# mkshing/e4t-diffusion

Hardware: AMD Instinct MI355X
Metric: E4T pretrain images/sec @512px bf16 (higher is better)
Workload: dtype bf16; 1 GPU; SD-1.4 UNet + ViT-H-14 E4T encoder pretrain step, 512px; per_gpu_batch=16, global_batch=16, parallelism=dp1, trainable=weight offsets + E4T head (ViT frozen), next_batch_prefetch=vit+vae

## Files before the change

e4t-diffusion_amd/csrc/common.h:

```cpp
#pragma once
#include <hip/hip_runtime.h>
#include <stdint.h>
#include <stdio.h>
#include <string.h>

typedef uint16_t bf16_t;

typedef __attribute__((ext_vector_type(8))) __bf16 bf16x8;
typedef __attribute__((ext_vector_type(4))) __bf16 bf16x4;
typedef __attribute__((ext_vector_type(16))) float f32x16;
typedef __attribute__((ext_vector_type(4))) float f32x4;

#define E4T_WAVE 64

typedef __attribute__((ext_vector_type(4))) short s16x4;
__device__ __forceinline__ bf16x8 tr_frag(const uint16_t* lds_lo, const uint16_t* lds_hi) {
  union { s16x4 h[2]; bf16x8 v; } u;
  u.h[0] = __builtin_amdgcn_ds_read_tr16_b64_v4i16((__attribute__((address_space(3))) s16x4*)lds_lo);
  u.h[1] = __builtin_amdgcn_ds_read_tr16_b64_v4i16((__attribute__((address_space(3))) s16x4*)lds_hi);
  return u.v;
}

extern "C" __attribute__((visibility("hidden"))) void e4t_set_error(const char* msg);
#define E4T_FAIL(code, ...)                                  \
  do {                                                       \
    char _b[512];                                            \
    snprintf(_b, sizeof(_b), __VA_ARGS__);                   \
    e4t_set_error(_b);                                       \
    return (code);                                           \
  } while (0)
#define E4T_REQUIRE(cond, ...) \
  do {                         \
    if (!(cond)) E4T_FAIL(-22, __VA_ARGS__); \
  } while (0)
#define E4T_CHECK_LAUNCH(name)                                                    \
  do {                                                                            \
    hipError_t _e = hipGetLastError();                                            \
    if (_e != hipSuccess) E4T_FAIL(-5, "%s: %s", name, hipGetErrorString(_e));    \
  } while (0)

extern "C" __attribute__((visibility("hidden"))) int e4t_launch_log_enabled(void);
extern "C" __attribute__((visibility("hidden"))) void e4t_launch_logf(const char* fmt, ...);
#define E4T_LOG_LAUNCH(...)                                          \
  do {                                                               \
    if (e4t_launch_log_enabled()) e4t_launch_logf(__VA_ARGS__);      \
  } while (0)

__device__ __forceinline__ float bf2f(bf16_t v) { return __uint_as_float(((uint32_t)v) << 16); }
typedef __attribute__((ext_vector_type(2))) __bf16 bf16x2_native;
typedef __attribute__((ext_vector_type(2))) float f32x2_native;
__device__ __forceinline__ bf16_t f2bf(float f) {
  const __bf16 b = (__bf16)f;
  bf16_t u;
  __builtin_memcpy(&u, &b, 2);
  return u;
}
__device__ __forceinline__ uint32_t pack2bf(float lo, float hi) {
  const f32x2_native f = {lo, hi};
  const bf16x2_native v = __builtin_convertvector(f, bf16x2_native);
  uint32_t u;
  __builtin_memcpy(&u, &v, 4);
  return u;
}
__device__ __forceinline__ float bflo(uint32_t w) { return __uint_as_float(w << 16); }
__device__ __forceinline__ float bfhi(uint32_t w) { return __uint_as_float(w & 0xffff0000u); }

__device__ __forceinline__ void unpack8(const uint4& v, float* f) {
  f[0] = bflo(v.x); f[1] = bfhi(v.x); f[2] = bflo(v.y); f[3] = bfhi(v.y);
  f[4] = bflo(v.z); f[5] = bfhi(v.z); f[6] = bflo(v.w); f[7] = bfhi(v.w);
}
__device__ __forceinline__ uint4 pack8(const float* f) {
  uint4 v;
  v.x = pack2bf(f[0], f[1]); v.y = pack2bf(f[2], f[3]); v.z = pack2bf(f[4], f[5]); v.w = pack2bf(f[6], f[7]);
  return v;
}
__device__ __forceinline__ void unpack4(const uint2& v, float* f) {
  f[0] = bflo(v.x); f[1] = bfhi(v.x); f[2] = bflo(v.y); f[3] = bfhi(v.y);
}
__device__ __forceinline__ uint2 pack4(const float* f) {
  uint2 v;
  v.x = pack2bf(f[0], f[1]); v.y = pack2bf(f[2], f[3]);
  return v;
}

__device__ __forceinline__ float wave_sum(float v) {
#pragma unroll
  for (int o = 32; o > 0; o >>= 1) v += __shfl_xor(v, o, 64);
  return v;
}
__device__ __forceinline__ float wave_max(float v) {
#pragma unroll
  for (int o = 32; o > 0; o >>= 1) v = fmaxf(v, __shfl_xor(v, o, 64));
  return v;
}
__device__ __forceinline__ float block_sum(float v, float* red) {
  v = wave_sum(v);
  const int w = threadIdx.x >> 6, nw = (blockDim.x + 63) >> 6;
  __syncthreads();
  if ((threadIdx.x & 63) == 0) red[w] = v;
  __syncthreads();
  float t = 0.f;
  for (int i = 0; i < nw; ++i) t += red[i];
  return t;
}

typedef __attribute__((ext_vector_type(4))) unsigned u32x4_native;
__device__ __forceinline__ uint4 buf_load16(__amdgpu_buffer_rsrc_t rs, unsigned voff, int soff) {
  const u32x4_native v = __builtin_amdgcn_raw_buffer_load_b128(rs, voff, soff, 0);
  return make_uint4(v.x, v.y, v.z, v.w);
}
__device__ __forceinline__ __amdgpu_buffer_rsrc_t make_rsrc(const void* base, unsigned bytes) {
  return __builtin_amdgcn_make_buffer_rsrc((void*)base, 0, (int)bytes, 0x00020000);
}

__device__ __forceinline__ float silu_f(float x) { return x / (1.f + __expf(-x)); }
__device__ __forceinline__ float dsilu_f(float x) {
  const float s = 1.f / (1.f + __expf(-x));
  return s * (1.f + x * (1.f - s));
}
__device__ __forceinline__ float erf_pos(float z, float e) {
  const float t = __builtin_amdgcn_rcpf(fmaf(0.3275911f, z, 1.f));
  float q = 1.061405429f;
  q = fmaf(q, t, -1.453152027f);
  q = fmaf(q, t, 1.421413741f);
  q = fmaf(q, t, -0.284496736f);
  q = fmaf(q, t, 0.254829592f);
  return fmaf(-q * t, e, 1.f);
}
__device__ __forceinline__ float gelu_f(float x) {
  const float e = __expf(-0.5f * x * x);
  const float er = erf_pos(fabsf(x) * 0.70710678118654752f, e);
  return 0.5f * x * (1.f + copysignf(er, x));
}
__device__ __forceinline__ float dgelu_f(float x) {
  const float e = __expf(-0.5f * x * x);
  const float er = erf_pos(fabsf(x) * 0.70710678118654752f, e);
  const float cdf = 0.5f * (1.f + copysignf(er, x));
  return fmaf(x * 0.39894228040143268f, e, cdf);
}

__device__ __forceinline__ float geglu_f(float a, float g) { return a * gelu_f(g); }
__device__ __forceinline__ float geglu_da_f(float d, float g) { return d * gelu_f(g); }
__device__ __forceinline__ float geglu_dg_f(float d, float a, float g) { return d * a * dgelu_f(g); }

static inline int cdiv(int a, int b) { return (a + b - 1) / b; }
static inline long long cdivl(long long a, long long b) { return (a + b - 1) / b; }
```

e4t-diffusion_amd/csrc/gemm.hip:

```cpp
#include "gemm_common.h"

namespace {


template <int BM, int BN, int WGM, int WGN, int MODE>
__global__ __launch_bounds__(256) void gemm_kernel(GemmArgs p) {
  constexpr int WM = BM / WGM, WN = BN / WGN;
  constexpr int FM = WM / 32, FN = WN / 32;
  constexpr int NA = BM * (BK / 8) / 256;
  constexpr int NB = BN * (BK / 8) / 256;
  static_assert(WGM * WGN == 4, "4 waves per workgroup");
  static_assert(NA >= 1 && NB >= 1, "tile too small");

  __shared__ __attribute__((aligned(16))) bf16_t smem[(BM + BN) * LDS_LD];
  bf16_t* const As = smem;
  bf16_t* const Bs = smem + BM * LDS_LD;

  const int tid = threadIdx.x;
  const int lane = tid & 63, wave = tid >> 6;
  const int wm = wave / WGN, wn = wave % WGN;
  const int m0 = blockIdx.y * BM, n0 = blockIdx.x * BN;

  const KRange kr = batch_entry<BK>(p, (p.K + BK - 1) / BK);
  const int kt_begin = kr.begin, kt_end = kr.end;
// ... 608 lines not shown
  wb.init(kt_begin, BK);
  int b_so = 0;
  int a_ky = (kt_begin % 9) / 3, a_chb = (kt_begin / 9) * BK * 2;
  auto issue_b = [&](bool hi, bf16_t* dst) __attribute__((always_inline)) {
    if (!hi) b_so = cm_b_so(p, wb);
    else b_so = __builtin_amdgcn_readfirstlane(b_so + HK * 2);
#pragma unroll
    for (int j = 0; j < 2; ++j) buf_dma16(rs_b, b_vo[j], b_so, dst + (wave * 32 + j * 16) * HK);
    if (hi) wb.next(BK);
  };
  auto issue_strip = [&](bool hi, bf16_t* dst) __attribute__((always_inline)) {
    const int iy = y + a_ky - 1;
    const int so = __builtin_amdgcn_readfirstlane((int)((((long long)ib * p.Hin + iy + 1) * p.Win + x0) * p.Cin * 2) + a_chb + (hi ? HK * 2 : 0));
#pragma unroll
    for (int i = 0; i < 3; ++i)
      buf_dma16(rs_a, a_vo[i] | (unsigned)__builtin_amdgcn_sbfe(a_inv[i], (unsigned)a_ky, 1u), so, dst + (wave + 8 * i) * 512);
    if (hi && ++a_ky == 3) { a_ky = 0; a_chb += BK * 2; }
  };
  auto issue_strip_piece = [&](auto Ic, bool last, bf16_t* dst_lo) __attribute__((always_inline)) {
    constexpr int i = decltype(Ic)::value;
    const int iy = y + a_ky - 1;
    const int so = __builtin_amdgcn_readfirstlane((int)((((long long)ib * p.Hin + iy + 1) * p.Win + x0) * p.Cin * 2) + a_chb);
    const unsigned vo = a_vo[i] | (unsigned)__builtin_amdgcn_sbfe(a_inv[i], (unsigned)a_ky, 1u);
    buf_dma16(rs_a, vo, so, dst_lo + (wave + 8 * i) * 512);
    buf_dma16(rs_a, vo, so + HK * 2, dst_lo + HSTRIP + (wave + 8 * i) * 512);
    if (last && ++a_ky == 3) { a_ky = 0; a_chb += BK * 2; }
  };

  f32x16 acc[4][2];
#pragma unroll
  for (int i = 0; i < 4; ++i)
#pragma unroll
    for (int j = 0; j < 2; ++j)
#pragma unroll
      for (int r = 0; r < 16; ++r) acc[i][j][r] = 0.f;

  const int frow = lane & 31, fhi = lane >> 5;
  int a_off[3][4][2], b_off[2][2];
#pragma unroll
  for (int ks = 0; ks < 2; ++ks) {
#pragma unroll
    for (int kx = 0; kx < 3; ++kx)
#pragma unroll
      for (int i = 0; i < 4; ++i) {
        const int o = wr * 128 + i * 32 + frow;
        const int r = sg.frag_row(o, kx);
        a_off[kx][i][ks] = frag_off<HK>(r, ks, fhi);
      }
#pragma unroll
    for (int j = 0; j < 2; ++j) {
      const int r = wc * 64 + j * 32 + frow;
      b_off[j][ks] = frag_off<HK>(r, ks, fhi);
    }
  }
  bf16_t* const Bq = smem + A_EL;
  issue_strip(false, smem);
  issue_strip(true, smem + HSTRIP);
  issue_b(false, Bq);
  issue_b(true, Bq + QUART);
  if (kt_begin + 1 < kt_end) issue_b(false, Bq + 2 * QUART);
  wait_vmcnt<0>();
  __builtin_amdgcn_s_barrier();

  bf16x8 af[2][2], bfr[2][2];
  using I0 = std::integral_constant<int, 0>; using I1 = std::integral_constant<int, 1>;
  using I2 = std::integral_constant<int, 2>; using I3 = std::integral_constant<int, 3>;
  auto phase = [&](auto Bc, auto Pc, auto ALLc, auto KXc, auto SPc, int kt) {
    constexpr int bb = decltype(Bc)::value, ph = decltype(Pc)::value, KX = decltype(KXc)::value, SP = decltype(SPc)::value;
    constexpr bool ALL = decltype(ALLc)::value;
    constexpr int kh = ph >> 1, mh = ph & 1;
    const bf16_t* const qa = smem + (2 * SP + kh) * HSTRIP;
    const bf16_t* const qb = Bq + (2 * bb + kh) * QUART;
#pragma unroll
    for (int i = 0; i < 2; ++i)
#pragma unroll
      for (int ks = 0; ks < 2; ++ks) af[i][ks] = *(const bf16x8*)(qa + a_off[KX][mh * 2 + i][ks]);
    if (mh == 0) {
#pragma unroll
      for (int j = 0; j < 2; ++j)
#pragma unroll
        for (int ks = 0; ks < 2; ++ks) bfr[j][ks] = *(const bf16x8*)(qb + b_off[j][ks]);
    }
    bool staged = true;
    if (ph == 0)      { staged = ALL || kt + 1 < kt_end; if (staged) issue_b(true, Bq + (2 * (bb ^ 1) + 1) * QUART); }
    else if (ph == 2) { staged = ALL || kt + 2 < kt_end; if (staged) issue_b(false, Bq + (2 * bb + 0) * QUART); }
    else if (4 * KX + ph == 1) { staged = ALL || kt + 3 < kt_end; if (staged) issue_strip_piece(I0{}, false, smem + 2 * (SP ^ 1) * HSTRIP); }
    else if (4 * KX + ph == 3) { staged = ALL || kt + 3 < kt_end; if (staged) issue_strip_piece(I1{}, false, smem + 2 * (SP ^ 1) * HSTRIP); }
    else if (4 * KX + ph == 5) { staged = ALL || kt + 2 < kt_end; if (staged) issue_strip_piece(I2{}, true, smem + 2 * (SP ^ 1) * HSTRIP); }
    constexpr int G_ = 4 * KX + ph;
    constexpr int NW_ = G_ == 0 ? 4 : G_ <= 2 ? 6 : G_ <= 6 ? 8 : G_ <= 8 ? 6 : 4;
    if (ALL || staged) wait_vmcnt<NW_>(); else wait_vmcnt<0>();
    __builtin_amdgcn_sched_barrier(0);
    __builtin_amdgcn_s_barrier();
    __builtin_amdgcn_sched_barrier(0);
    __builtin_amdgcn_s_setprio(1);
#pragma unroll
    for (int ks = 0; ks < 2; ++ks)
#pragma unroll
      for (int i = 0; i < 2; ++i)
#pragma unroll
        for (int j = 0; j < 2; ++j)
          acc[mh * 2 + i][j] = __builtin_amdgcn_mfma_f32_32x32x16_bf16(af[i][ks], bfr[j][ks], acc[mh * 2 + i][j], 0, 0, 0);
    __builtin_amdgcn_s_setprio(0);
    __builtin_amdgcn_sched_barrier(0);
    __builtin_amdgcn_s_barrier();
    __builtin_amdgcn_sched_barrier(0);
  };
  auto ktile = [&](auto Bc, auto KXc, auto SPc, auto ALLc, int kt) __attribute__((always_inline)) {
    phase(Bc, I0{}, ALLc, KXc, SPc, kt); phase(Bc, I1{}, ALLc, KXc, SPc, kt); phase(Bc, I2{}, ALLc, KXc, SPc, kt); phase(Bc, I3{}, ALLc, KXc, SPc, kt);
  };

  if (wr == 1) __builtin_amdgcn_s_barrier();
  {
    using YES = std::true_type; using NO = std::false_type;
    int kt = kt_begin;
    for (; kt + 8 <= kt_end; kt += 6) {
      ktile(I0{}, I0{}, I0{}, YES{}, kt);     ktile(I1{}, I1{}, I0{}, YES{}, kt + 1); ktile(I0{}, I2{}, I0{}, YES{}, kt + 2);
      ktile(I1{}, I0{}, I1{}, YES{}, kt + 3); ktile(I0{}, I1{}, I1{}, YES{}, kt + 4); ktile(I1{}, I2{}, I1{}, YES{}, kt + 5);
    }
    if (kt < kt_end) { ktile(I0{}, I0{}, I0{}, NO{}, kt); ktile(I1{}, I1{}, I0{}, NO{}, kt + 1); ktile(I0{}, I2{}, I0{}, NO{}, kt + 2); kt += 3; }
    if (kt < kt_end) { ktile(I1{}, I0{}, I1{}, NO{}, kt); ktile(I0{}, I1{}, I1{}, NO{}, kt + 1); ktile(I1{}, I2{}, I1{}, NO{}, kt + 2); kt += 3; }
  }
  if (wr == 0) __builtin_amdgcn_s_barrier();
  __syncthreads();
  write_tile<64, 64, 2, 2, GENERAL>(p, *(f32x16(*)[2][2])(acc + 0), wave_stage<64, 64>(smem, wave), lane, m0 + wr * 128, n0 + wc * 64);
  __syncthreads();
  write_tile<64, 64, 2, 2, GENERAL>(p, *(f32x16(*)[2][2])(acc + 2), wave_stage<64, 64>(smem, wave), lane, m0 + wr * 128 + 64, n0 + wc * 64);
}
static bool conv_pps_ok(const GemmArgs& p, int , int batch) {
  return strips_enabled() && p.mode == E4T_CONV_S1 && p.chan_major && batch == 1 && strip_rows_ok(p) && p.Wout == p.Win && p.Hout == p.Hin && p.Cin % 64 == 0 &&
         p.K == 9 * p.Cin && p.ktiles_per_split % 3 == 0 && p.M % 256 == 0;
}

template <int MODE, int BN, bool GENERAL>
__global__ __launch_bounds__(512) void gemm_pq_kernel(GemmArgs p) {
  constexpr int EPI = EPI_PLAIN;
#include "gemm_pq_kernel.inc"
}
template <int BN, int EPI>
__global__ __launch_bounds__(512) void gemm_pq_geglu_kernel(GemmArgs p) {
  constexpr int MODE = 0;
  constexpr bool GENERAL = false;
#include "gemm_pq_kernel.inc"
}

#ifdef PP_TRACE
}
extern "C" int e4t_debug_pp_trace(unsigned long long* out) {
  return (int)hipMemcpyFromSymbol(out, HIP_SYMBOL(g_pp_trace), sizeof(g_pp_trace));
}
namespace {
#endif

__global__ __launch_bounds__(512) void gemm_tn_kernel(GemmArgs p) {
  constexpr int BM = 128, BN = 128, WGN = 2, WM = 32, WN = 64, FN = 2;
  constexpr int OPER = BK * 128;
  constexpr int TILE = 2 * OPER;
  __shared__ __attribute__((aligned(16))) bf16_t smem[2 * TILE];

  const int tid = threadIdx.x;
  const int lane = tid & 63, wave = __builtin_amdgcn_readfirstlane(tid >> 6);
  const int wm = wave / WGN, wn = wave % WGN;
  int tile_x, tile_y, sz = blockIdx.z;
  if (p.xcd3) { xcd_tile3(tile_x, tile_y, sz); p.zslab = sz; }
  else xcd_tile(tile_x, tile_y, p.group_m);
  const int m0 = tile_y * BM, n0 = tile_x * BN;

  const int nkt = (p.K + BK - 1) / BK;
  const int kt_begin = sz * p.ktiles_per_split;
  int kt_end = kt_begin + p.ktiles_per_split;
  if (kt_end > nkt) kt_end = nkt;

  const __amdgpu_buffer_rsrc_t rs_a = __builtin_amdgcn_make_buffer_rsrc((void*)p.A, 0, (int)p.a_bytes, 0x00020000);
  const __amdgpu_buffer_rsrc_t rs_b = __builtin_amdgcn_make_buffer_rsrc((void*)p.B, 0, (int)p.b_bytes, 0x00020000);
  const int prow = lane >> 4, pchunk = lane & 15;
  const int lchunk = (((pchunk >> 1) ^ (2 * prow)) << 1) | (pchunk & 1);
  const bool a_col_ok = m0 + lchunk * 8 < p.M, b_col_ok = n0 + lchunk * 8 < p.N;
  unsigned a_col[2], b_col[2], a_vo[2], b_vo[2];
#pragma unroll
  for (int i = 0; i < 2; ++i) {
    const int r = (wave * 2 + i) * 4 + prow;
    a_col[i] = a_col_ok ? (unsigned)(((size_t)r * p.lda + m0 + lchunk * 8) * 2) : OOB;
    b_col[i] = b_col_ok ? (unsigned)(((size_t)r * p.ldb + n0 + lchunk * 8) * 2) : OOB;
  }
  int a_so = 0, b_so = 0;
  auto issue_tile = [&](int kt, bf16_t* buf) __attribute__((always_inline)) {
    if (kt == kt_begin || (kt + 1) * BK > p.K) {
      a_so = kt * BK * p.lda * 2; b_so = kt * BK * p.ldb * 2;
#pragma unroll
      for (int i = 0; i < 2; ++i) {
        const bool row_ok = kt * BK + (wave * 2 + i) * 4 + prow < p.K;
        a_vo[i] = row_ok ? a_col[i] : OOB;
        b_vo[i] = row_ok ? b_col[i] : OOB;
      }
    } else {
      a_so += BK * p.lda * 2; b_so += BK * p.ldb * 2;
    }
#pragma unroll
    for (int i = 0; i < 2; ++i) buf_dma16(rs_a, a_vo[i], a_so, buf + (wave * 2 + i) * 512);
#pragma unroll
    for (int i = 0; i < 2; ++i) buf_dma16(rs_b, b_vo[i], b_so, buf + OPER + (wave * 2 + i) * 512);
  };

  f32x16 acc[1][FN];
#pragma unroll
  for (int j = 0; j < FN; ++j)
#pragma unroll
    for (int r = 0; r < 16; ++r) acc[0][j][r] = 0.f;

  const int g16 = lane >> 4, il = lane & 15;
  const int frow = (g16 >> 1) * 8 + (il >> 2);
  auto frag_off = [&](int col0) {
    const int col = col0 + 16 * (g16 & 1) + 4 * (il & 3);
    const int unit = (col >> 4) ^ (2 * (il >> 2));
    return frow * 128 + unit * 16 + (col & 15);
  };
  const int a_off = frag_off(wm * WM);
  int b_off[FN];
#pragma unroll
  for (int j = 0; j < FN; ++j) b_off[j] = OPER + frag_off(wn * WN + j * 32);

  if (kt_begin < kt_end) issue_tile(kt_begin, smem);
  auto body = [&](auto CURc, int kt) {
    constexpr int CUR = decltype(CURc)::value;
    wait_vmcnt<0>();
    loop_barrier();
    const bf16_t* st = smem + CUR * TILE;
    bf16x8 af[2], bfr[2][FN];
    af[0] = tr_frag(st + a_off, st + a_off + 512);
#pragma unroll
    for (int j = 0; j < FN; ++j) bfr[0][j] = tr_frag(st + b_off[j], st + b_off[j] + 512);
    if (kt + 1 < kt_end) issue_tile(kt + 1, smem + (CUR ^ 1) * TILE);
#pragma unroll
    for (int ks = 0; ks < BK / 16; ++ks) {
      const int c = ks & 1, n = c ^ 1;
      if (ks + 1 < BK / 16) {
        af[n] = tr_frag(st + a_off + (ks + 1) * 2048, st + a_off + (ks + 1) * 2048 + 512);
#pragma unroll
        for (int j = 0; j < FN; ++j) bfr[n][j] = tr_frag(st + b_off[j] + (ks + 1) * 2048, st + b_off[j] + (ks + 1) * 2048 + 512);
      }
#pragma unroll
      for (int j = 0; j < FN; ++j) acc[0][j] = __builtin_amdgcn_mfma_f32_32x32x16_bf16(af[c], bfr[c][j], acc[0][j], 0, 0, 0);
    }
  };
  {
    int kt = kt_begin;
    for (; kt + 2 <= kt_end; kt += 2) {
      body(std::integral_constant<int, 0>{}, kt);
      body(std::integral_constant<int, 1>{}, kt + 1);
    }
    if (kt < kt_end) body(std::integral_constant<int, 0>{}, kt);
  }
  __syncthreads();
  write_tile<WM, WN, 1, FN>(p, acc, wave_stage<WM, WN>(smem, wave), lane, m0 + wm * WM, n0 + wn * WN);
}

__global__ __launch_bounds__(256) void splitk_reduce_kernel(GemmArgs p, int nz) {
  const size_t total = (size_t)p.M * p.N;
  const int bz = blockIdx.y;
  if (!p.reduce_batch) {
    if (p.bias) p.bias += bz * p.strideBias;
    if (p.flags & E4T_OUT_F32) p.C = (float*)p.C + bz * p.strideC;
    else p.C = (bf16_t*)p.C + bz * p.strideC;
  }
  const float* ws = p.ws + (size_t)bz * nz * total;
  for (size_t idx = (size_t)blockIdx.x * 256 + threadIdx.x; idx < total; idx += (size_t)gridDim.x * 256) {
    float v = 0.f;
    for (int z = 0; z < nz; ++z) v += ws[(size_t)z * total + idx];
    const int row = (int)(idx / p.N), col = (int)(idx - (size_t)row * p.N);
    epilogue_store(p, v, row, col);
  }
}

__global__ __launch_bounds__(256) void splitk_reduce8_kernel(GemmArgs p, int nz) {
  const int n8 = p.N >> 3;
  const size_t total = (size_t)p.M * p.N, total8 = (size_t)p.M * n8;
  const int bz = blockIdx.y;
  if (!p.reduce_batch) {
    if (p.bias) p.bias += bz * p.strideBias;
    p.C = (bf16_t*)p.C + bz * p.strideC;
  }
  const float* ws = p.ws + (size_t)bz * nz * total;
  const bf16_t* Rb = (const bf16_t*)p.residual;
  for (size_t i8 = (size_t)blockIdx.x * 256 + threadIdx.x; i8 < total8; i8 += (size_t)gridDim.x * 256) {
    const int row = (int)(i8 / n8), c8 = (int)(i8 - (size_t)row * n8) * 8;
    const size_t idx = (size_t)row * p.N + c8;
    float bi[8] = {0.f, 0.f, 0.f, 0.f, 0.f, 0.f, 0.f, 0.f}, rb[8] = {0.f, 0.f, 0.f, 0.f, 0.f, 0.f, 0.f, 0.f}, rs[8] = {0.f, 0.f, 0.f, 0.f, 0.f, 0.f, 0.f, 0.f};
    if (p.bias) { const float4 a = *(const float4*)(p.bias + c8), b = *(const float4*)(p.bias + c8 + 4); bi[0] = a.x; bi[1] = a.y; bi[2] = a.z; bi[3] = a.w; bi[4] = b.x; bi[5] = b.y; bi[6] = b.z; bi[7] = b.w; }
    if (p.rowbias) {
      const float* q = p.rowbias + (size_t)(row / p.rows_per_batch) * p.ldrb + c8;
      const float4 a = *(const float4*)q, b = *(const float4*)(q + 4);
      rb[0] = a.x; rb[1] = a.y; rb[2] = a.z; rb[3] = a.w; rb[4] = b.x; rb[5] = b.y; rb[6] = b.z; rb[7] = b.w;
    }
    if (Rb) unpack8(*(const uint4*)(Rb + (size_t)row * p.ldr + c8), rs);
    float v[8] = {0.f, 0.f, 0.f, 0.f, 0.f, 0.f, 0.f, 0.f};
    for (int z0 = 0; z0 < nz; z0 += 4) {
      float4 lo[4], hi[4];
#pragma unroll
      for (int u = 0; u < 4; ++u) {
        const float* q = ws + (size_t)min(z0 + u, nz - 1) * total + idx;
        lo[u] = *(const float4*)q; hi[u] = *(const float4*)(q + 4);
      }
#pragma unroll
      for (int u = 0; u < 4; ++u) {
        const float w = z0 + u < nz ? 1.f : 0.f;
        v[0] += lo[u].x * w; v[1] += lo[u].y * w; v[2] += lo[u].z * w; v[3] += lo[u].w * w;
        v[4] += hi[u].x * w; v[5] += hi[u].y * w; v[6] += hi[u].z * w; v[7] += hi[u].w * w;
      }
    }
#pragma unroll
    for (int k = 0; k < 8; ++k) {
      float x = v[k] * p.alpha + bi[k] + rb[k];
      if (p.flags & E4T_ACT_GELU) x = gelu_f(x);
      v[k] = x + rs[k];
    }
    *(uint4*)((bf16_t*)p.C + (size_t)row * p.ldc + c8) = pack8(v);
  }
}

__global__ __launch_bounds__(256) void splitk_reduce4f_kernel(GemmArgs p, int nz) {
  const int n4 = p.N >> 2;
  const size_t total = (size_t)p.M * p.N, total4 = (size_t)p.M * n4;
  const int bz = blockIdx.y;
  float* Cf = (float*)p.C + (p.reduce_batch ? 0 : bz * p.strideC);
  const float* ws = p.ws + (size_t)bz * nz * total;
  for (size_t i4 = (size_t)blockIdx.x * 256 + threadIdx.x; i4 < total4; i4 += (size_t)gridDim.x * 256) {
    const int row = (int)(i4 / n4), c4 = (int)(i4 - (size_t)row * n4) * 4;
    const size_t idx = (size_t)row * p.N + c4;
    float4 v = make_float4(0.f, 0.f, 0.f, 0.f);
    for (int z0 = 0; z0 < nz; z0 += 8) {
      float4 t[8];
#pragma unroll
      for (int u = 0; u < 8; ++u) t[u] = *(const float4*)(ws + (size_t)min(z0 + u, nz - 1) * total + idx);
#pragma unroll
      for (int u = 0; u < 8; ++u) {
        const float w = z0 + u < nz ? 1.f : 0.f;
        v.x += t[u].x * w; v.y += t[u].y * w; v.z += t[u].z * w; v.w += t[u].w * w;
      }
    }
    float4* c = (float4*)(Cf + (size_t)row * p.ldc + c4);
    float4 o = make_float4(v.x * p.alpha, v.y * p.alpha, v.z * p.alpha, v.w * p.alpha);
    if (p.flags & E4T_ACCUM) { const float4 a = *c; o.x += a.x; o.y += a.y; o.z += a.z; o.w += a.w; }
    *c = o;
  }
}

int device_cu_count() {
  static const int ncu = [] {
    int dev = 0, n = 0;
    return hipGetDevice(&dev) == hipSuccess && hipDeviceGetAttribute(&n, hipDeviceAttributeMultiprocessorCount, dev) == hipSuccess && n > 0 ? n : 256;
  }();
  return ncu;
}

bool dma_allowed() { static const bool on = getenv("E4T_GEMM_REGSTAGE") == nullptr; return on; }
struct KernelEntry { void (*fn)(GemmArgs); const char* text; int threads; };
#define KERNEL(threads, name, ...) {&name<__VA_ARGS__>, #name "<" #__VA_ARGS__ ">", threads}
#define NO_KERNEL {nullptr, nullptr, 0}
enum : unsigned {
  CAP_STAGED = 1u << 0,
  CAP_BUF = 1u << 1,
  CAP_COLSTATS = 1u << 2,
  CAP_SPLITK = 1u << 3,
  CAP_WHOLE_K = 1u << 4,
  CAP_WHOLE_N = 1u << 5,
  CAP_TAIL = 1u << 6,
  CAP_PANELS = 1u << 7,
  CAP_ONE_PER_CU = 1u << 8,
  CAP_GEGLU = 1u << 9,
  CAP_DMA = CAP_BUF | CAP_COLSTATS | CAP_SPLITK,
};
struct StripAlt { bool (*ok)(const GemmArgs&, int, int); KernelEntry k[2]; };
struct Variant {
  int tile, kt, stages, tm, tn;
  unsigned caps;
  KernelEntry gemm[2], conv[2], conv_cm[2];
  StripAlt alt;
  KernelEntry geglu[2];
};

#define DMA_FN(nt, bm, bn, wgm, wgn, st, kt) {KERNEL(nt, gemm_dma_kernel, bm, bn, wgm, wgn, 0, st, false, kt), NO_KERNEL}, \
                                             {KERNEL(nt, gemm_dma_kernel, bm, bn, wgm, wgn, 1, st, false, kt), NO_KERNEL}
#define DMA_FN_GENERAL(nt, bm, bn, wgm, wgn, st)                                                                                  \
  {KERNEL(nt, gemm_dma_kernel, bm, bn, wgm, wgn, 0, st, false, 64), KERNEL(nt, gemm_dma_kernel, bm, bn, wgm, wgn, 0, st, true, 64)}, \
  {KERNEL(nt, gemm_dma_kernel, bm, bn, wgm, wgn, 1, st, false, 64), KERNEL(nt, gemm_dma_kernel, bm, bn, wgm, wgn, 1, st, true, 64)}
#define DMA_GEGLU(nt, bm, bn, wgm, wgn, st, kt) {KERNEL(nt, gemm_dma_geglu_kernel, bm, bn, wgm, wgn, st, kt, 1), KERNEL(nt, gemm_dma_geglu_kernel, bm, bn, wgm, wgn, st, kt, 2)}
#define DMA_GEGLU_F(nt, bm, bn, wgm, wgn, st, kt) {KERNEL(nt, gemm_dma_geglu_kernel, bm, bn, wgm, wgn, st, kt, 1), NO_KERNEL}
#define DMA_GEGLU_B(nt, bm, bn, wgm, wgn, st, kt) {NO_KERNEL, KERNEL(nt, gemm_dma_geglu_kernel, bm, bn, wgm, wgn, st, kt, 2)}
#define REG_FN(bm, bn, mode) {{&gemm_kernel<bm, bn, 2, 2, mode>, "gemm_kernel", 256}, {&gemm_kernel<bm, bn, 2, 2, mode>, "gemm_kernel", 256}}
static const Variant kVariants[] = {
    {64, 64, 2, 64, 64, CAP_DMA | CAP_STAGED, DMA_FN_GENERAL(256, 64, 64, 2, 2, 2)},
    {64, 64, 3, 64, 64, CAP_DMA | CAP_STAGED | CAP_GEGLU, DMA_FN_GENERAL(256, 64, 64, 2, 2, 3), {}, {}, DMA_GEGLU_F(256, 64, 64, 2, 2, 3, 64)},
    {64, 64, 4, 64, 64, CAP_DMA | CAP_STAGED | CAP_GEGLU, DMA_FN(256, 64, 64, 2, 2, 4, 64), {}, {}, DMA_GEGLU_B(256, 64, 64, 2, 2, 4, 64)},
    {128, 64, 2, 128, 128, CAP_DMA | CAP_STAGED | CAP_GEGLU, DMA_FN_GENERAL(512, 128, 128, 4, 2, 2), {}, {}, DMA_GEGLU(512, 128, 128, 4, 2, 2, 64)},
    {128, 64, 3, 128, 128, CAP_DMA | CAP_STAGED, DMA_FN(512, 128, 128, 4, 2, 3, 64)},
    {128, 64, 4, 128, 128, CAP_DMA | CAP_STAGED | CAP_GEGLU, DMA_FN(512, 128, 128, 4, 2, 4, 64), {}, {}, DMA_GEGLU_B(512, 128, 128, 4, 2, 4, 64)},
    {160, 64, 2, 128, 160, CAP_DMA | CAP_STAGED | CAP_TAIL | CAP_GEGLU, DMA_FN_GENERAL(256, 128, 160, 4, 1, 2), {}, {}, DMA_GEGLU_F(256, 128, 160, 4, 1, 2, 64)},
    {160, 64, 3, 128, 160, CAP_DMA | CAP_STAGED | CAP_TAIL | CAP_GEGLU, DMA_FN(256, 128, 160, 4, 1, 3, 64), {}, {}, DMA_GEGLU_B(256, 128, 160, 4, 1, 3, 64)},
    {160, 64, 4, 128, 160, CAP_DMA | CAP_STAGED | CAP_TAIL, DMA_FN(256, 128, 160, 4, 1, 4, 64)},
    {256, 32, 3, 256, 128, CAP_DMA | CAP_GEGLU, DMA_FN(512, 256, 128, 4, 2, 3, 32), {}, {conv_strip_ok, {KERNEL(512, conv_strip_kernel, 2), NO_KERNEL}},
     DMA_GEGLU(512, 256, 128, 4, 2, 3, 32)},
    {512, 64, 2, 256, 256, CAP_DMA | CAP_WHOLE_K | CAP_TAIL | CAP_ONE_PER_CU,
     {KERNEL(512, gemm_pp_kernel, 0, false, false), KERNEL(512, gemm_pp_kernel, 0, true, false)},
     {KERNEL(512, gemm_pp_kernel, 1, false, false), KERNEL(512, gemm_pp_kernel, 1, true, false)},
     {KERNEL(512, gemm_pp_kernel, 1, false, true), KERNEL(512, gemm_pp_kernel, 1, true, true)},
     {conv_pps_ok, {KERNEL(512, gemm_pps_kernel, false), KERNEL(512, gemm_pps_kernel, true)}}},
    {2320, 64, 2, 256, 320, CAP_DMA | CAP_WHOLE_K | CAP_WHOLE_N | CAP_TAIL | CAP_PANELS | CAP_ONE_PER_CU | CAP_GEGLU,
// ... 329 lines not shown
void fill_gemm_args(const e4t_gemm_desc* d, GemmArgs& p) {
  memset(&p, 0, sizeof(p));
  p.zslab = -1;
  p.A = (const bf16_t*)d->A; p.A2 = (const bf16_t*)d->A2; p.K1 = d->A2 ? d->K1 : d->K; p.lda = d->lda; p.lda2 = d->lda2;
  p.B = (const bf16_t*)d->B; p.ldb = d->ldb; p.C = d->C; p.ldc = d->ldc; p.bias = d->bias; p.residual = d->residual; p.ldr = d->ldr;
  p.rowbias = d->rowbias; p.rows_per_batch = d->rows_per_batch > 0 ? d->rows_per_batch : 1; p.ldrb = d->ldrb > 0 ? d->ldrb : d->N;
  p.M = d->M; p.N = d->N; p.K = d->K; p.alpha = d->alpha; p.flags = d->flags; p.ws = (float*)d->workspace;
  p.strideA = d->strideA; p.strideB = d->strideB; p.strideC = d->strideC; p.strideBias = d->strideBias;
  p.reduce_batch = (d->flags & E4T_REDUCE_BATCH) ? 1 : 0;
  p.colstats = d->colstats;
  p.panel_rows = d->panel_rows; p.panel_stride = d->panel_stride; p.panel_off = d->panel_off;
  p.aux = d->aux; p.ldaux = d->ldaux;
}

int check_conv_geometry(const e4t_conv_desc* d) {
  const int Cin = d->Cin, Cout = d->Cout, Hin = d->Hin, Win = d->Win, Hout = d->Hout, Wout = d->Wout, mode = d->mode;
  E4T_REQUIRE(Cin % BK == 0, "conv3x3: Cin=%d must be a multiple of 64 (pad the input channels)", Cin);
  E4T_REQUIRE(mode >= E4T_CONV_S1 && mode <= E4T_CONV_S2A, "conv3x3: bad mode %d", mode);
  E4T_REQUIRE(d->B > 0 && Hin > 0 && Win > 0 && Hout > 0 && Wout > 0 && Cout > 0, "conv3x3: bad geometry");
  if (mode == E4T_CONV_S1) E4T_REQUIRE(Hout == Hin && Wout == Win, "conv3x3 S1: output must equal input size");
  if (mode == E4T_CONV_S2) E4T_REQUIRE(Hout == (Hin - 1) / 2 + 1 && Wout == (Win - 1) / 2 + 1, "conv3x3 S2: bad output size");
  if (mode == E4T_CONV_UP2) E4T_REQUIRE(Hout == 2 * Hin && Wout == 2 * Win, "conv3x3 UP2: output must be 2x input");
  if (mode == E4T_CONV_S2T) E4T_REQUIRE(Hin == (Hout - 1) / 2 + 1 && Win == (Wout - 1) / 2 + 1, "conv3x3 S2T: bad sizes");
  if (mode == E4T_CONV_S2A) E4T_REQUIRE(Hout == (Hin - 2) / 2 + 1 && Wout == (Win - 2) / 2 + 1, "conv3x3 S2A: bad output size");
  return 0;
}

void fill_conv_args(const e4t_conv_desc* d, GemmArgs& p) {
  const int Cin = d->Cin, Cout = d->Cout;
  memset(&p, 0, sizeof(p));
  p.zslab = -1;
  p.A = (const bf16_t*)d->X; p.K1 = 9 * Cin; p.Hin = d->Hin; p.Win = d->Win; p.Cin = Cin; p.Hout = d->Hout; p.Wout = d->Wout;
  p.mode = d->mode; p.B = (const bf16_t*)d->W; p.ldb = 9 * Cin; p.C = d->Y; p.ldc = Cout; p.bias = d->bias;
  p.residual = d->residual; p.ldr = Cout; p.rowbias = d->rowbias; p.rows_per_batch = d->Hout * d->Wout; p.ldrb = d->ldrb > 0 ? d->ldrb : Cout;
  p.M = d->B * d->Hout * d->Wout; p.N = Cout; p.K = 9 * Cin; p.alpha = 1.f; p.flags = d->flags; p.ws = (float*)d->workspace;
  p.colstats = d->colstats;
}

int tn_splitk(int M, int N, int K, int req) {
  const int nkt = cdiv(K, BK);
  const long long tiles = (long long)cdiv(N, 128) * cdiv(M, 128);
  int splitk = req;
  if (splitk <= 0) {
    splitk = (int)(512 / tiles);
    if (splitk > 32) splitk = 32;
    if (splitk > nkt / 16) splitk = nkt / 16;
    if (splitk < 1) splitk = 1;
  }
  if (splitk > nkt) splitk = nkt;
  return cdiv(nkt, cdiv(nkt, splitk));
}

void export_plan(const GemmPlan& pl, const GemmArgs& p, int batch, e4t_gemm_plan_t* out, int tail = 0) {
  out->tile = pl.kt32 ? 5000 + pl.tile : pl.tile; out->tile_m = pl.shape->tm; out->tile_n = pl.shape->tn; out->splitk = pl.splitk;
  out->workspace_bytes = (pl.splitk > 1 || p.reduce_batch) ? (size_t)pl.splitk * batch * p.M * p.N * sizeof(float) : 0;
  out->tail_rows = tail; out->stages = (!pl.kt32 && (pl.shape->caps & CAP_STAGED)) ? pl.stages : 0;
}

}

extern "C" int e4t_gemm_plan(const e4t_gemm_desc* d, e4t_gemm_plan_t* out) {
  E4T_REQUIRE(d && out && d->M > 0 && d->N > 0 && d->K > 0, "gemm_plan: bad arguments");
  GemmArgs p;
  fill_gemm_args(d, p);
  const int batch = d->batch > 0 ? d->batch : 1;
  int tail = 0;
  const GemmPlan pl = plan_gemm_tail(p, false, d->tile, d->splitk, batch, tail);
  export_plan(pl, p, batch, out, tail);
  E4T_REFUSE_FUSED(pl, p, tail, batch);
  return 0;
}

extern "C" int e4t_conv3x3_plan(const e4t_conv_desc* d, e4t_gemm_plan_t* out) {
  E4T_REQUIRE(d && out && d->B > 0 && d->Hout > 0 && d->Wout > 0 && d->Cin > 0 && d->Cout > 0, "conv3x3_plan: bad arguments");
  GemmArgs p;
  fill_conv_args(d, p);
  export_plan(plan_gemm(p, true, d->tile, d->splitk, 1), p, 1, out);
  return 0;
}

extern "C" int e4t_gemm_tn_plan(const e4t_gemm_desc* d, e4t_gemm_plan_t* out) {
  E4T_REQUIRE(d && out && d->M > 0 && d->N > 0 && d->K > 0, "gemm_tn_plan: bad arguments");
  out->tile = 128; out->tile_m = out->tile_n = 128; out->tail_rows = out->stages = 0;
  out->splitk = tn_splitk(d->M, d->N, d->K, d->splitk);
  out->workspace_bytes = out->splitk > 1 ? (size_t)out->splitk * d->M * d->N * sizeof(float) : 0;
  return 0;
}

extern "C" int e4t_gemm_nt(const e4t_gemm_desc* d, e4t_stream stream) {
  E4T_REQUIRE(d && d->A && d->B && d->C, "gemm_nt: null operand");
  E4T_REQUIRE(d->M > 0 && d->N > 0 && d->K > 0, "gemm_nt: bad shape M=%d N=%d K=%d", d->M, d->N, d->K);
  E4T_REQUIRE(d->K % 8 == 0 && d->lda % 8 == 0 && d->ldb % 8 == 0, "gemm_nt: K, lda, ldb must be multiples of 8 (16-B rows)");
  E4T_REQUIRE(((uintptr_t)d->A & 15) == 0 && ((uintptr_t)d->B & 15) == 0, "gemm_nt: A/B must be 16-B aligned");
  if (d->A2) {
    E4T_REQUIRE(d->K1 % BK == 0 && d->K1 > 0 && d->K1 < d->K && d->lda2 % 8 == 0 && ((uintptr_t)d->A2 & 15) == 0,
                "gemm_nt: two-source A needs K1 %% 64 == 0, 0 < K1 < K");
  }
  E4T_REQUIRE(!d->rowbias || d->rows_per_batch > 0, "gemm_nt: rowbias needs rows_per_batch");
  const int batch = d->batch > 0 ? d->batch : 1;
  E4T_REQUIRE(batch == 1 || (d->strideA % 8 == 0 && d->strideB % 8 == 0), "gemm_nt: batch strides must keep 16-B alignment");
  E4T_REQUIRE(!(d->flags & E4T_REDUCE_BATCH) || !d->A2, "gemm_nt: reduce-batch with two-source A unsupported");
  if (d->panel_rows) {
    E4T_REQUIRE(d->panel_rows > 0 && d->panel_rows % 256 == 0 && d->panel_stride >= d->panel_rows && d->panel_off >= 0 && d->M % d->panel_rows == 0,
                "gemm_nt: row panels need panel_rows %% 256 == 0, panel_stride >= panel_rows, M %% panel_rows == 0");
    E4T_REQUIRE(batch == 1 && !d->rowbias && !d->colstats && !d->A2 && !(d->flags & (E4T_ACCUM | E4T_REDUCE_BATCH)) && d->splitk <= 1,
                "gemm_nt: row panels do not combine with batch / row bias / column statistics / two-source A / accumulate / split-K");
  }
  E4T_REQUIRE(!(d->flags & (E4T_EPI_GEGLU | E4T_EPI_GEGLU_BWD)) || d->aux, "gemm_nt: the fused GEGLU epilogues need aux (h out / u in)");
  GemmArgs p;
  fill_gemm_args(d, p);
  return launch_gemm(p, false, d->tile, d->workspace_bytes, d->splitk, batch, (hipStream_t)stream);
}

extern "C" int e4t_gemm_tn(const e4t_gemm_desc* d, e4t_stream stream) {
  E4T_REQUIRE(d && d->A && d->B && d->C, "gemm_tn: null operand");
  E4T_REQUIRE(d->M > 0 && d->N > 0 && d->K > 0 && d->batch <= 1 && !d->A2 && !d->rowbias, "gemm_tn: bad / unsupported arguments");
  E4T_REQUIRE(!(d->flags & (E4T_ACT_GELU | E4T_EPI_GEGLU | E4T_EPI_GEGLU_BWD)), "gemm_tn: the GELU / GEGLU epilogues are not built for the TN kernel");
  E4T_REQUIRE(d->M % 8 == 0 && d->N % 8 == 0 && d->lda % 8 == 0 && d->ldb % 8 == 0 && ((uintptr_t)d->A & 15) == 0 && ((uintptr_t)d->B & 15) == 0,
              "gemm_tn: M, N, lda, ldb must be multiples of 8 and the operands 16-byte aligned");
  GemmArgs p;
  memset(&p, 0, sizeof(p));
  p.zslab = -1;
  p.A = (const bf16_t*)d->A; p.lda = d->lda; p.B = (const bf16_t*)d->B; p.ldb = d->ldb;
  p.C = d->C; p.ldc = d->ldc; p.bias = d->bias; p.residual = d->residual; p.ldr = d->ldr;
  p.M = d->M; p.N = d->N; p.K = d->K; p.K1 = d->K; p.alpha = d->alpha; p.flags = d->flags & ~E4T_REDUCE_BATCH;
  p.rows_per_batch = 1; p.ldrb = d->N;
  p.ws = (float*)d->workspace;
  const int nkt = cdiv(p.K, BK), gx = cdiv(p.N, 128), gy = cdiv(p.M, 128);
  {
    const unsigned long long ab = ((unsigned long long)(p.K - 1) * p.lda + p.M) * 2, bb = ((unsigned long long)(p.K - 1) * p.ldb + p.N) * 2;
    E4T_REQUIRE(ab < 0xFFFF0000ull && bb < 0xFFFF0000ull, "gemm_tn: operands beyond 4 GB are not supported");
    p.a_bytes = (unsigned)ab; p.b_bytes = (unsigned)bb;
  }
  int splitk = tn_splitk(p.M, p.N, p.K, d->splitk);
  p.ktiles_per_split = cdiv(nkt, splitk);
  const size_t need = (size_t)splitk * p.M * p.N * sizeof(float);
  if (splitk > 1 && (p.ws == nullptr || d->workspace_bytes < need)) {
    if (d->splitk > 1) E4T_FAIL(-12, "gemm_tn: split-K=%d needs %zu workspace bytes, have %zu", splitk, need, d->workspace_bytes);
    splitk = 1;
    p.ktiles_per_split = nkt;
  }
  if (splitk <= 1) p.ws = nullptr;
  p.splitk = splitk;
  p.group_m = 8;
  p.xcd3 = splitk > 1;
  p.fast_epi = bf16_rows_aligned16(p);
  hipStream_t st = (hipStream_t)stream;
  if (e4t_launch_log_enabled()) {
    const double osz = (p.flags & E4T_OUT_F32) ? 4.0 : 2.0;
    E4T_LOG_LAUNCH("gemm_tn_kernel|gemm_tn M%d N%d K%d splitk%d flags%d|%.0f|%.0f", p.M, p.N, p.K, splitk, p.flags,
                   2.0 * (double)p.K * (p.M + p.N) + osz * (double)p.M * p.N * ((p.flags & E4T_ACCUM) ? 2 : 1), 2.0 * p.M * p.N * (double)p.K);
    if (p.ws) log_splitk_reduce(p, splitk, splitk, false);
  }
  hipLaunchKernelGGL(gemm_tn_kernel, dim3(gx, gy, splitk), dim3(512), 0, st, p);
  E4T_CHECK_LAUNCH("gemm_tn_kernel");
  return p.ws ? launch_splitk_reduce(p, splitk, 1, false, st) : 0;
}

extern "C" int e4t_conv3x3(const e4t_conv_desc* d, e4t_stream stream) {
  E4T_REQUIRE(d && d->X && d->W && d->Y, "conv3x3: null operand");
  if (const int rc = check_conv_geometry(d); rc < 0) return rc;
  GemmArgs p;
  fill_conv_args(d, p);
  return launch_gemm(p, true, d->tile, d->workspace_bytes, d->splitk, 1, (hipStream_t)stream);
}

extern "C" int e4t_conv3x3_kernel(const e4t_conv_desc* d, const char** symbol, int* splitk) {
  E4T_REQUIRE(d && symbol && splitk, "conv3x3_kernel: bad arguments");
  if (const int rc = check_conv_geometry(d); rc < 0) return rc;
  GemmArgs p;
  fill_conv_args(d, p);
  int tail = 0;
  const GemmPlan pl = plan_gemm_tail(p, true, d->tile, d->splitk, 1, tail);
  const KernelEntry* entry = nullptr;
  const int sk = resolve_launch(pl, p, true, EPI_PLAIN, d->workspace_bytes, d->splitk, 1, entry);
  if (sk < 0) return sk;
  *symbol = entry->text;
  *splitk = sk;
  return 0;
}
```

Measured before the change: 157.5 images/s.

## Restructure TN GEMM into 4-stage pipelined 256-thread kernel with batched transposed LDS reads

The TN GEMM kernel (used for weight gradients) drops from 512 to 256 threads, and each wave now computes a 64x64 tile (2x2 MFMA fragments) instead of 32x64. The K loop is split into 32-deep half-stages held in a 4-buffer LDS ring with a lookahead of 3, so the global wait uses partial vmcnt counts instead of draining fully. Transposed LDS reads are issued eight at a time through inline asm with explicit lgkmcnt waits, overlapping the second k-step's reads with the first step's MFMAs. An f32 direct-store epilogue for split-K partials and plain f32 outputs is also added. These changes aim to raise reuse per wave and hide memory latency, at the cost of more registers per wave and fewer waves per block.

```diff
diff --git a/e4t-diffusion_amd/csrc/common.h b/e4t-diffusion_amd/csrc/common.h
--- a/e4t-diffusion_amd/csrc/common.h
+++ b/e4t-diffusion_amd/csrc/common.h
@@ -19,6 +19,34 @@
   u.h[0] = __builtin_amdgcn_ds_read_tr16_b64_v4i16((__attribute__((address_space(3))) s16x4*)lds_lo);
   u.h[1] = __builtin_amdgcn_ds_read_tr16_b64_v4i16((__attribute__((address_space(3))) s16x4*)lds_hi);
   return u.v;
+}
+
+struct TrFrags {
+  s16x4 r[8];
+  __device__ __forceinline__ bf16x8 a(int i) const { union { s16x4 h[2]; bf16x8 v; } u; u.h[0] = r[2 * i]; u.h[1] = r[2 * i + 1]; return u.v; }
+  __device__ __forceinline__ bf16x8 b(int j) const { union { s16x4 h[2]; bf16x8 v; } u; u.h[0] = r[4 + 2 * j]; u.h[1] = r[5 + 2 * j]; return u.v; }
+};
+template <int OFF>
+__device__ __forceinline__ void tr_read_frags(TrFrags& f, unsigned a0, unsigned a1, unsigned b0, unsigned b1) {
+  static_assert(OFF >= 0 && OFF + 1024 < 65536, "ds offset field");
+  asm volatile(
+      "ds_read_b64_tr_b16 %0, %8 offset:%12\n\t"
+      "ds_read_b64_tr_b16 %1, %8 offset:%13\n\t"
+      "ds_read_b64_tr_b16 %2, %9 offset:%12\n\t"
+      "ds_read_b64_tr_b16 %3, %9 offset:%13\n\t"
+      "ds_read_b64_tr_b16 %4, %10 offset:%12\n\t"
+      "ds_read_b64_tr_b16 %5, %10 offset:%13\n\t"
+      "ds_read_b64_tr_b16 %6, %11 offset:%12\n\t"
+      "ds_read_b64_tr_b16 %7, %11 offset:%13"
+      : "=&v"(f.r[0]), "=&v"(f.r[1]), "=&v"(f.r[2]), "=&v"(f.r[3]), "=&v"(f.r[4]), "=&v"(f.r[5]), "=&v"(f.r[6]), "=&v"(f.r[7])
+      : "v"(a0), "v"(a1), "v"(b0), "v"(b1), "n"(OFF), "n"(OFF + 1024)
+      : "memory");
+}
+__device__ __forceinline__ void tr_wait_frags(TrFrags& f) {
+  asm volatile("s_waitcnt lgkmcnt(0)"
+               : "+v"(f.r[0]), "+v"(f.r[1]), "+v"(f.r[2]), "+v"(f.r[3]), "+v"(f.r[4]), "+v"(f.r[5]), "+v"(f.r[6]), "+v"(f.r[7])
+               :
+               : "memory");
 }
 
 extern "C" __attribute__((visibility("hidden"))) void e4t_set_error(const char* msg);
diff --git a/e4t-diffusion_amd/csrc/gemm.hip b/e4t-diffusion_amd/csrc/gemm.hip
--- a/e4t-diffusion_amd/csrc/gemm.hip
+++ b/e4t-diffusion_amd/csrc/gemm.hip
@@ -784,11 +784,45 @@
 namespace {
 #endif
 
-__global__ __launch_bounds__(512) void gemm_tn_kernel(GemmArgs p) {
-  constexpr int BM = 128, BN = 128, WGN = 2, WM = 32, WN = 64, FN = 2;
-  constexpr int OPER = BK * 128;
-  constexpr int TILE = 2 * OPER;
-  __shared__ __attribute__((aligned(16))) bf16_t smem[2 * TILE];
+template <int FM, int FN>
+__device__ __forceinline__ void tn_store_f32(const GemmArgs& p, f32x16 (&acc)[FM][FN], int lane, int mw, int nw) {
+  const bool partial = p.ws != nullptr;
+  float* base = partial ? p.ws + (size_t)(p.zslab >= 0 ? p.zslab : (int)blockIdx.z) * p.M * p.N : (float*)p.C;
+  const int ld = partial ? p.N : p.ldc;
+  const float alpha = partial ? 1.f : p.alpha;
+  const bool accum = !partial && (p.flags & E4T_ACCUM) != 0;
+  const int frow = lane & 31, fhi = lane >> 5;
+#pragma unroll
+  for (int i = 0; i < FM; ++i)
+#pragma unroll
+    for (int j = 0; j < FN; ++j) {
+      const int col = nw + j * 32 + frow, colc = min(col, p.N - 1);
+      float old[16];
+      if (accum) {
+#pragma unroll
+        for (int r = 0; r < 16; ++r) {
+          const int row = min(mw + i * 32 + (r & 3) + 8 * (r >> 2) + 4 * fhi, p.M - 1);
+          old[r] = base[(size_t)row * ld + colc];
+        }
+      }
+#pragma unroll
+      for (int r = 0; r < 16; ++r) {
+        const int row = mw + i * 32 + (r & 3) + 8 * (r >> 2) + 4 * fhi;
+        float v = acc[i][j][r] * alpha;
+        if (accum) v += old[r];
+        if (row < p.M && col < p.N) base[(size_t)row * ld + col] = v;
+      }
+      __builtin_amdgcn_sched_barrier(0);
+    }
+}
+
+__global__ __launch_bounds__(256) void gemm_tn_kernel(GemmArgs p) {
+  constexpr int BM = 128, BN = 128, WGN = 2, WM = 64, WN = 64, FM = 2, FN = 2;
+  constexpr int HK = 32;
+  constexpr int OPER = HK * 128;
+  constexpr int STAGE = 2 * OPER;
+  constexpr int NSTAGE = 4, LOOK = 3, P = 4;
+  __shared__ __attribute__((aligned(16))) bf16_t smem[NSTAGE * STAGE];
 
   const int tid = threadIdx.x;
   const int lane = tid & 63, wave = __builtin_amdgcn_readfirstlane(tid >> 6);
@@ -798,10 +832,10 @@
   else xcd_tile(tile_x, tile_y, p.group_m);
   const int m0 = tile_y * BM, n0 = tile_x * BN;
 
-  const int nkt = (p.K + BK - 1) / BK;
-  const int kt_begin = sz * p.ktiles_per_split;
-  int kt_end = kt_begin + p.ktiles_per_split;
-  if (kt_end > nkt) kt_end = nkt;
+  const int nh = (p.K + HK - 1) / HK;
+  const int h_begin = sz * p.ktiles_per_split * (BK / HK);
+  int h_end = h_begin + p.ktiles_per_split * (BK / HK);
+  if (h_end > nh) h_end = nh;
 
   const __amdgpu_buffer_rsrc_t rs_a = __builtin_amdgcn_make_buffer_rsrc((void*)p.A, 0, (int)p.a_bytes, 0x00020000);
   const __amdgpu_buffer_rsrc_t rs_b = __builtin_amdgcn_make_buffer_rsrc((void*)p.B, 0, (int)p.b_bytes, 0x00020000);
@@ -816,17 +850,17 @@
     b_col[i] = b_col_ok ? (unsigned)(((size_t)r * p.ldb + n0 + lchunk * 8) * 2) : OOB;
   }
   int a_so = 0, b_so = 0;
-  auto issue_tile = [&](int kt, bf16_t* buf) __attribute__((always_inline)) {
-    if (kt == kt_begin || (kt + 1) * BK > p.K) {
-      a_so = kt * BK * p.lda * 2; b_so = kt * BK * p.ldb * 2;
+  auto issue_stage = [&](int h, bf16_t* buf) __attribute__((always_inline)) {
+    if (h == h_begin || (h + 1) * HK > p.K) {
+      a_so = h * HK * p.lda * 2; b_so = h * HK * p.ldb * 2;
 #pragma unroll
       for (int i = 0; i < 2; ++i) {
-        const bool row_ok = kt * BK + (wave * 2 + i) * 4 + prow < p.K;
+        const bool row_ok = h * HK + (wave * 2 + i) * 4 + prow < p.K;
         a_vo[i] = row_ok ? a_col[i] : OOB;
         b_vo[i] = row_ok ? b_col[i] : OOB;
       }
     } else {
-      a_so += BK * p.lda * 2; b_so += BK * p.ldb * 2;
+      a_so += HK * p.lda * 2; b_so += HK * p.ldb * 2;
     }
 #pragma unroll
     for (int i = 0; i < 2; ++i) buf_dma16(rs_a, a_vo[i], a_so, buf + (wave * 2 + i) * 512);
@@ -834,11 +868,13 @@
     for (int i = 0; i < 2; ++i) buf_dma16(rs_b, b_vo[i], b_so, buf + OPER + (wave * 2 + i) * 512);
   };
 
-  f32x16 acc[1][FN];
-#pragma unroll
-  for (int j = 0; j < FN; ++j)
-#pragma unroll
-    for (int r = 0; r < 16; ++r) acc[0][j][r] = 0.f;
+  f32x16 acc[FM][FN];
+#pragma unroll
+  for (int i = 0; i < FM; ++i)
+#pragma unroll
+    for (int j = 0; j < FN; ++j)
+#pragma unroll
+      for (int r = 0; r < 16; ++r) acc[i][j][r] = 0.f;
 
   const int g16 = lane >> 4, il = lane & 15;
   const int frow = (g16 >> 1) * 8 + (il >> 2);
@@ -847,44 +883,60 @@
     const int unit = (col >> 4) ^ (2 * (il >> 2));
     return frow * 128 + unit * 16 + (col & 15);
   };
-  const int a_off = frag_off(wm * WM);
-  int b_off[FN];
-#pragma unroll
-  for (int j = 0; j < FN; ++j) b_off[j] = OPER + frag_off(wn * WN + j * 32);
-
-  if (kt_begin < kt_end) issue_tile(kt_begin, smem);
-  auto body = [&](auto CURc, int kt) {
+  static_assert(FM == 2 && FN == 2 && HK == 32, "tr_read_frags gathers 2 + 2 operands; a stage is two k-steps");
+  const unsigned lds0 = (unsigned)(size_t)(__attribute__((address_space(3))) bf16_t*)smem;
+  unsigned a_lds[FM], b_lds[FN];
+#pragma unroll
+  for (int i = 0; i < FM; ++i) a_lds[i] = lds0 + 2 * frag_off(wm * WM + i * 32);
+#pragma unroll
+  for (int j = 0; j < FN; ++j) b_lds[j] = lds0 + 2 * (OPER + frag_off(wn * WN + j * 32));
+
+#pragma unroll
+  for (int s = 0; s < LOOK; ++s)
+    if (h_begin + s < h_end) issue_stage(h_begin + s, smem + s * STAGE);
+
+  auto body = [&](auto CURc, int h) {
     constexpr int CUR = decltype(CURc)::value;
-    wait_vmcnt<0>();
+    constexpr int NXT = (CUR + LOOK) % NSTAGE;
+    if (h + 2 < h_end) wait_vmcnt<2 * P>();
+    else if (h + 1 < h_end) wait_vmcnt<P>();
+    else wait_vmcnt<0>();
     loop_barrier();
-    const bf16_t* st = smem + CUR * TILE;
-    bf16x8 af[2], bfr[2][FN];
-    af[0] = tr_frag(st + a_off, st + a_off + 512);
-#pragma unroll
-    for (int j = 0; j < FN; ++j) bfr[0][j] = tr_frag(st + b_off[j], st + b_off[j] + 512);
-    if (kt + 1 < kt_end) issue_tile(kt + 1, smem + (CUR ^ 1) * TILE);
-#pragma unroll
-    for (int ks = 0; ks < BK / 16; ++ks) {
-      const int c = ks & 1, n = c ^ 1;
-      if (ks + 1 < BK / 16) {
-        af[n] = tr_frag(st + a_off + (ks + 1) * 2048, st + a_off + (ks + 1) * 2048 + 512);
-#pragma unroll
-        for (int j = 0; j < FN; ++j) bfr[n][j] = tr_frag(st + b_off[j] + (ks + 1) * 2048, st + b_off[j] + (ks + 1) * 2048 + 512);
-      }
-#pragma unroll
-      for (int j = 0; j < FN; ++j) acc[0][j] = __builtin_amdgcn_mfma_f32_32x32x16_bf16(af[c], bfr[c][j], acc[0][j], 0, 0, 0);
-    }
+    TrFrags f0, f1;
+    tr_read_frags<CUR * STAGE * 2>(f0, a_lds[0], a_lds[1], b_lds[0], b_lds[1]);
+    if (h + LOOK < h_end) issue_stage(h + LOOK, smem + NXT * STAGE);
+    tr_wait_frags(f0);
+    tr_read_frags<CUR * STAGE * 2 + 4096>(f1, a_lds[0], a_lds[1], b_lds[0], b_lds[1]);
+    __builtin_amdgcn_sched_barrier(0);
+#pragma unroll
+    for (int i = 0; i < FM; ++i)
+#pragma unroll
+      for (int j = 0; j < FN; ++j) acc[i][j] = __builtin_amdgcn_mfma_f32_32x32x16_bf16(f0.a(i), f0.b(j), acc[i][j], 0, 0, 0);
+    __builtin_amdgcn_sched_barrier(0);
+    tr_wait_frags(f1);
+#pragma unroll
+    for (int i = 0; i < FM; ++i)
+#pragma unroll
+      for (int j = 0; j < FN; ++j) acc[i][j] = __builtin_amdgcn_mfma_f32_32x32x16_bf16(f1.a(i), f1.b(j), acc[i][j], 0, 0, 0);
   };
   {
-    int kt = kt_begin;
-    for (; kt + 2 <= kt_end; kt += 2) {
-      body(std::integral_constant<int, 0>{}, kt);
-      body(std::integral_constant<int, 1>{}, kt + 1);
-    }
-    if (kt < kt_end) body(std::integral_constant<int, 0>{}, kt);
+    int h = h_begin;
+    for (; h + NSTAGE <= h_end; h += NSTAGE) {
+      body(std::integral_constant<int, 0>{}, h);
+      body(std::integral_constant<int, 1>{}, h + 1);
+      body(std::integral_constant<int, 2>{}, h + 2);
+      body(std::integral_constant<int, 3>{}, h + 3);
+    }
+    if (h < h_end) { body(std::integral_constant<int, 0>{}, h); ++h; }
+    if (h < h_end) { body(std::integral_constant<int, 1>{}, h); ++h; }
+    if (h < h_end) { body(std::integral_constant<int, 2>{}, h); ++h; }
+  }
+  if (p.ws || ((p.flags & E4T_OUT_F32) && !p.bias && !p.residual)) {
+    tn_store_f32<FM, FN>(p, acc, lane, m0 + wm * WM, n0 + wn * WN);
+    return;
   }
   __syncthreads();
-  write_tile<WM, WN, 1, FN>(p, acc, wave_stage<WM, WN>(smem, wave), lane, m0 + wm * WM, n0 + wn * WN);
+  write_tile<WM, WN, FM, FN>(p, acc, wave_stage<WM, WN>(smem, wave), lane, m0 + wm * WM, n0 + wn * WN);
 }
 
 __global__ __launch_bounds__(256) void splitk_reduce_kernel(GemmArgs p, int nz) {
@@ -1520,7 +1572,7 @@
                    2.0 * (double)p.K * (p.M + p.N) + osz * (double)p.M * p.N * ((p.flags & E4T_ACCUM) ? 2 : 1), 2.0 * p.M * p.N * (double)p.K);
     if (p.ws) log_splitk_reduce(p, splitk, splitk, false);
   }
-  hipLaunchKernelGGL(gemm_tn_kernel, dim3(gx, gy, splitk), dim3(512), 0, st, p);
+  hipLaunchKernelGGL(gemm_tn_kernel, dim3(gx, gy, splitk), dim3(256), 0, st, p);
   E4T_CHECK_LAUNCH("gemm_tn_kernel");
   return p.ws ? launch_splitk_reduce(p, splitk, 1, false, st) : 0;
 }
```

Result: no change. 158.5 images/s, median of 6 (+0.6%).
